# antrea-io/theia

Hardware: AMD Instinct MI355X
Metric: flow-records/sec (higher is better)
Workload: dtype u64 (aggregates) + f64 (detectors)

## Files before the change

### theia_amd/_capi.py

```python
import ctypes as C
import os

from . import build as _build

u64, i64, i32, u32, f64, f32 = C.c_uint64, C.c_int64, C.c_int32, C.c_uint32, C.c_double, C.c_float

TAD_ABI_VERSION = 13
TAD_KEY_SKIP = (1 << 64) - 1
TAD_OK = 0
TAD_ERR_INVALID_ARGUMENT, TAD_ERR_NO_DEVICE, TAD_ERR_OUT_OF_MEMORY, TAD_ERR_HIP = -1, -2, -3, -4
TAD_ERR_KEY_RANGE, TAD_ERR_GRID_TOO_LARGE, TAD_ERR_BUSY = -5, -6, -7
TAD_ALGO = {"EWMA": 0, "ARIMA": 1, "DBSCAN": 2, "DROP": 3}
TAD_AGG = {"": 0, None: 0, "None": 0, "pod": 1, "svc": 2, "external": 3}
TAD_OP = {"auto": 0, "max": 1, "sum": 2}
TAD_MEM_HOST, TAD_MEM_DEVICE = 0, 1
TAD_FLAG_EMIT_ALL_POINTS = 1
TAD_FLAG_KEY_U32, TAD_FLAG_TIME_U32 = 2, 4
TAD_KEY_SKIP32 = (1 << 32) - 1
TAD_FEATURE_NARROW_COLUMNS = 1
TAD_FEATURE_STREAM_DBSCAN = 2
TAD_STATE_HISTORY = 1
TAD_FEATURE_STREAM_ARIMA = 4
TAD_STATE_SERIES = 2
TAD_FEATURE_STREAM_TRIM = 8
TAD_STATE_TIMES = 8
TAD_FEATURE_STATE_RUN = 16
TAD_FEATURE_STATE_MERGE = 32
TAD_FEATURE_STATE_WINDOW = 64


class Plan(C.Structure):
    _fields_ = [("stage0", i32), ("partition_pass", i32), ("histogram", i32), ("sparse", i32), ("sparse_classes", i32),
                ("ewma_emit", i32), ("ewma_emit_rows", u32), ("reserved0", i32), ("tile_cells", i32), ("sparse_sort", i32), ("reserved1", i32)]


PLAN_VALUES = {
    "stage0": {"auto": 0, "v1": 1, "v2": 2}, "partition_pass": {"auto": 0, "sort": 1, "wc": 2, "wc_sectors": 3}, "histogram": {"auto": 0, "exact": 1, "sampled": 2},
    "sparse": {"auto": 0, "never": 1, "always": 2}, "sparse_classes": {"auto": 0, "always": 1}, "ewma_emit": {"auto": 0, "staged": 0, "lane": 1}, "tile_cells": {"auto": 0, "wide": 1},
    "sparse_sort": {"auto": 0, "lsd": 1, "partition": 2},
}


def make_plan(**kw):
    p = Plan()
    for name, v in kw.items():
        if name not in dict((f[0], 1) for f in Plan._fields_):
            raise ValueError("unknown tad_plan field %r" % name)
        if isinstance(v, str):
            v = PLAN_VALUES[name][v]
        setattr(p, name, int(v))
    return p


class KeyColumns(C.Structure):
    _fields_ = [("n_rows", u64), ("n_cols", i32), ("cols_a", C.POINTER(C.c_void_p)), ("keep_a", C.c_void_p),
                ("cols_b", C.POINTER(C.c_void_p)), ("keep_b", C.c_void_p), ("memory", C.c_int)]


class StringColumn(C.Structure):
    _fields_ = [("n_rows", u64), ("offsets", C.c_void_p), ("offset_bits", i32), ("data", C.c_void_p), ("data_bytes", u64),
                ("validity", C.c_void_p), ("validity_offset", u64), ("memory", C.c_int)]
# ... 136 lines not shown
```

### theia_amd/csrc/tad_capi.cpp

```cpp
#include "tad_engine.h"

using namespace tad;
using namespace tadh;

namespace tadh {

int ensure_rcp_table(JobCtx *e, uint64_t T) {
  const uint64_t want = T + 2;
  if (want <= e->rcp_n) return TAD_OK;
  uint64_t cap = want < 1024 ? 1024 : want + want / 4;
  int rc = ensure(e, e->rcp_table, cap * sizeof(double));
  if (rc != TAD_OK) return rc;
  std::vector<double> h(cap);
  h[0] = 0.0;
  for (uint64_t i = 1; i < cap; ++i) h[i] = 1.0 / (double)i;
  HIP_TRY(e, hipMemcpyAsync(e->rcp_table.p, h.data(), cap * sizeof(double), hipMemcpyHostToDevice, e->stream));
  HIP_TRY(e, hipStreamSynchronize(e->stream));
  e->rcp_n = cap;
  return TAD_OK;
}

int ensure_key_buffers(JobCtx *e, uint64_t K) {
  int rc;
  const uint64_t k = K ? K : 1;
// ... 24 lines not shown
    while (__atomic_load_n(&e->eng->pause_count, __ATOMIC_ACQUIRE) != 0 && std::chrono::steady_clock::now() - t0 < std::chrono::milliseconds(2))
      std::this_thread::sleep_for(std::chrono::microseconds(50));
    const uint32_t grace = __atomic_load_n(&e->eng->pause_count, __ATOMIC_ACQUIRE) != 0 ? 24u : 0u;
    if (relaunch(grace, &yielded_dev) != 0) return fail(e, TAD_ERR_HIP, "ARIMA launch failed");
    e->arima_relaunches++;
  }
  return TAD_OK;
}

int detect_and_count(JobCtx *e, Grid g, JobParams &jp, DevCounters *ctr, uint64_t *rows, bool stats_done = false) {
  hipStream_t s = e->stream;
  int rc;
  if ((rc = ensure_key_buffers(e, g.K)) != TAD_OK) return rc;
  if ((rc = ensure_rcp_table(e, g.T)) != TAD_OK) return rc;
  double *sigma = static_cast<double *>(e->sigma.p);
  uint32_t *n_pts = static_cast<uint32_t *>(e->n_pts.p);
  uint32_t *n_anom = static_cast<uint32_t *>(e->n_anom.p);
  unsigned long long *off = static_cast<unsigned long long *>(e->off.p);

  const bool ewma = jp.algo == TAD_ALGO_EWMA;
  const bool drop = jp.algo == TAD_ALGO_DROP;
  const bool db_fused = jp.algo == TAD_ALGO_DBSCAN && !jp.all_points && !stats_done && dbscan_uses_list(g);
  jp.lazy_sigma = db_fused;
  if (drop) {
    if ((rc = ensure(e, e->calc, (g.K * g.T ? g.K * g.T : 1) * sizeof(double))) != TAD_OK) return rc;
    launch_drop(s, g, jp.drop_nsigma, jp.drop_min_samples, static_cast<double *>(e->calc.p), sigma, n_pts,
                static_cast<double *>(e->key_mean.p), static_cast<double *>(e->key_m2.p), ctr);
  } else if (!stats_done && !db_fused)
    launch_key_sigma(s, g, jp.alpha, ewma && !jp.all_points, static_cast<const double *>(e->rcp_table.p), sigma, n_pts, n_anom, ctr, static_cast<double *>(e->key_mean.p),
                     static_cast<double *>(e->key_m2.p));
  if (jp.algo == TAD_ALGO_DBSCAN) {
    if ((rc = ensure(e, e->aux, dbscan_scratch_bytes(g))) != TAD_OK) return rc;
    if (dbscan_uses_list(g)) {
      DbscanStats dst{nullptr, nullptr, nullptr, nullptr};
      if (db_fused) dst = DbscanStats{n_pts, n_anom, static_cast<double *>(e->key_mean.p), static_cast<double *>(e->key_m2.p)};
      if (launch_dbscan(s, g, jp.eps, jp.min_samples, e->aux.p, dst, jp.settled && db_fused) != 0)
        return fail(e, TAD_ERR_HIP, "DBSCAN launch failed");
    } else {
      return fail(e, TAD_ERR_GRID_TOO_LARGE, "DBSCAN: series of %llu buckets are not supported", (unsigned long long)g.T);
    }
  } else if (jp.algo == TAD_ALGO_ARIMA) {
    if ((rc = ensure(e, e->calc, g.K * g.T * sizeof(double))) != TAD_OK) return rc;
    const size_t wsb = arima_workspace_bytes(g);
    if ((rc = ensure(e, e->aux, wsb)) != TAD_OK) return rc;
    const bool held = e->hold && e->hold->held;
    if (held) e->hold->release();
    const unsigned int *yielded_dev = nullptr;
    if (launch_arima(s, g, sigma, n_pts, jp.maxiter, static_cast<double *>(e->calc.p), ctr, e->aux.p, wsb, e->eng->pause_dev, &yielded_dev) != 0)
      return fail(e, TAD_ERR_HIP, "ARIMA launch failed");
    if ((rc = arima_yield_loop(e, yielded_dev, [&](uint32_t grace, const unsigned int **yd) {
           return launch_arima_fit(s, g, sigma, n_pts, jp.maxiter, static_cast<double *>(e->calc.p), ctr, e->aux.p, e->eng->pause_dev, yd, grace);
         })) != TAD_OK)
      return rc;
    if (held) e->hold->acquire();
  }
  const uint32_t *cnt = n_anom;
  if (jp.all_points && jp.algo != TAD_ALGO_ARIMA && !drop) cnt = n_pts;
  else if (db_fused) {}
  else if (!ewma || jp.all_points) launch_count_flags(s, g, jp.all_points, n_anom);
  launch_scan_moments(s, cnt, off, g.K, static_cast<unsigned long long *>(e->scan_scratch.p), dev_total(e), n_pts,
                      static_cast<const double *>(e->key_mean.p), static_cast<const double *>(e->key_m2.p), dev_moments(e), db_fused ? ctr : nullptr);
  HIP_TRY(e, hipMemcpyAsync(e->tail_host, e->counters.p, kTailBytes, hipMemcpyDeviceToHost, s));
  HIP_TRY(e, hipStreamSynchronize(s));
  HIP_TRY(e, hipGetLastError());
  *rows = *e->total_host;
  return TAD_OK;
}

}

namespace tadh {

void emit_rows(JobCtx *e, Grid g, Lattice L, const JobParams &jp, OutRows out, uint64_t rows) {
  const int kind = jp.algo == TAD_ALGO_EWMA ? 0 : (jp.algo == TAD_ALGO_ARIMA ? 1 : (jp.algo == TAD_ALGO_DROP ? 3 : (jp.lazy_sigma ? 4 : 2)));
  if (kind == 4 && !jp.all_points &&
      launch_emit_dbscan_list(e->stream, g, L, e->aux.p, static_cast<const uint32_t *>(e->n_anom.p), static_cast<const unsigned long long *>(e->off.p), out))
    return;
  launch_emit(e->stream, g, L, kind, jp.all_points, jp.alpha, static_cast<const double *>(e->sigma.p),
              static_cast<const uint32_t *>(e->n_pts.p), static_cast<const double *>(kind == 3 ? e->key_mean.p : e->calc.p),
              static_cast<const unsigned long long *>(e->off.p), out, rows, e->plan.ewma_emit, e->plan.ewma_emit_rows);
}

}

namespace {

int make_result(JobCtx *e, uint64_t rows, bool with_anomaly, tad_mem out_memory, ResultPriv **out, OutRows *dev_rows,
                ResultBlock *dev_block) {
  ResultPriv *rp = new (std::nothrow) ResultPriv();
  if (!rp) return fail(e, TAD_ERR_OUT_OF_MEMORY, "out of host memory");
  memset(rp, 0, sizeof *rp);
  const size_t bytes = result_bytes(rows, with_anomaly);
  int rc = alloc_device_block(e, bytes, dev_block);
  if (rc != TAD_OK) { delete rp; return rc; }
  carve(dev_block->base, rows, with_anomaly, dev_rows);
  rp->pub.n_rows = rows;
  rp->pub.memory = out_memory;
  *out = rp;
  return TAD_OK;
}
// ... 682 lines not shown
  HIP_TRY(e, hipEventRecord(e->ev[0], s));
  if (depth == 0) HIP_TRY(e, hipEventRecord(e->ev[6], s));
  int lat_mode = cols->n_buckets > 0 ? 0 : 1;
  Lattice L = make_lattice(cols->t0, lat_mode == 0 ? cols->step : 1, cols->n_buckets);
  bool empty = (n == 0 || K == 0);
  const tad_plan plan = e->plan;
  const bool force_v1 = plan.stage0 == 1;
  const bool force_v2 = plan.stage0 == 2;
  const bool has2 = cols->key_id2 != nullptr;
  bool force_v1_retry = false;
  bool force_wide_tiles = plan.tile_cells == 1;
  bool force_exact_hist = plan.histogram == 1;
  bool learnt_exact_hist = false, probing_sampled_hist = false;
  bool kh_rejected = false;
  bool sparse_lsd = plan.sparse_sort == 1;
  {
    const JobCtx::Learnt &lt = e->learnt;
    if (depth == 0 && lt.valid && lt.n == n && lt.K == K && lt.has2 == has2 && lt.algo == (int)job->algo && lt.op == (int)op_max) {
      if (lt.exact_hist) {
        if (lt.exact_uses >= lt.exact_backoff) probing_sampled_hist = true;
        else { force_exact_hist = true; learnt_exact_hist = true; }
      }
      if (lt.wide_tiles) force_wide_tiles = true;
    }
  }
  for (int attempt = 0; attempt < 11; ++attempt) {
    const bool hinted = lat_mode == 0;
    HIP_TRY(e, hipMemsetAsync(ctr, 0, kTailMoments, s));
    jp.settled = false;
    bool narrow_tiles = false;
    PartPlan pl{};
    bool v2 = !empty && !force_v1 && !force_v1_retry && (force_v2 || n >= (1ull << 22)) && part_plan_bins(n, K, has2, &pl);
    if (v2 && e->hold) e->hold->acquire();
    if ((rc = ensure(e, e->meta, sizeof(MetaPartial) * kMetaBlocks)) != TAD_OK) return rc;
    int meta_blocks = 0;
    bool hist_sampled = false;
    const tad_key_hist *kh = cols->key_hist;
    bool use_kh = v2 && depth == 0 && !kh_rejected && kh != nullptr && kh->bins != nullptr && lat_mode != 2 && kh->n_rows == n && kh->num_keys == K &&
                  kh->sides == (has2 ? 2u : 1u) && kh->workgroups == (uint32_t)pl.G && kh->nbins == pl.nbins && kh->shift == (uint32_t)pl.shift_bin &&
                  kh->chunk_rows == pl.chunk && rf.end_time == 0 && !(d_ts != nullptr && rf.start_time != 0);
    const uint32_t *binhist = nullptr;
    if (v2) {
      if ((rc = ensure(e, e->binhist, (size_t)pl.G * pl.nbins * 4)) != TAD_OK) return rc;
      hist_sampled = launch_meta_hist(s, (const uint64_t *)d_key, (const uint64_t *)d_key2, (const int64_t *)d_te, (const int64_t *)d_ts, n, K, rf,
                                      pl, static_cast<MetaPartial *>(e->meta.p), static_cast<uint32_t *>(e->binhist.p), ctr, cw,
                                      use_kh ||
// ... 495 lines not shown
        for (uint64_t i = 0; i < rows; ++i) st.n_anomalies += a[i];
      }
    }
    hipEventElapsedTime(&st.ms_meta, e->ev[0], e->ev[1]);
    hipEventElapsedTime(&st.ms_stage0, e->ev[1], e->ev[5]);
    hipEventElapsedTime(&st.ms_scatter, e->ev[2], e->ev[3]);
    hipEventElapsedTime(&st.ms_detect, e->ev[5], e->ev[4]);
    st.stage0_path = sparse ? (sp_part ? 8 : 4) : (v2 ? (pl.wc_cap ? 3 : 2) : 1);
    st.stage0_attempts = attempt + 1;
    st.hist_sampled = (v2 && hist_sampled) ? 1 : (use_kh ? 2 : 0);
    st.host_syncs = (hinted || empty) ? 2 : 3;
    st.job_context = e->index;
    st.arima_relaunches = e->arima_relaunches;
    hipEventElapsedTime(&st.ms_total, e->ev[0], e->ev[4]);
    if (depth == 0 && !points_mode && !stream) {
      JobCtx::Learnt &w = e->learnt;
      const bool exact_now = force_exact_hist && plan.histogram != 1;
      if (learnt_exact_hist) w.exact_uses++;
      else if (probing_sampled_hist) { w.exact_uses = 0; w.exact_backoff = exact_now ? (w.exact_backoff < 64 ? w.exact_backoff * 2 : 64) : 8; }
      else { w.exact_uses = 0; w.exact_backoff = 8; }
      w.valid = true; w.n = n; w.K = K; w.has2 = has2; w.algo = (int)job->algo; w.op = (int)op_max;
      w.exact_hist = exact_now;
      w.wide_tiles = force_wide_tiles && plan.tile_cells != 1;
    }
    strncpy(rp->pub.id, job->id, sizeof rp->pub.id - 1);
    if (stream && g.K) {
      unsigned long long added = 0;
      memcpy(&added, e->tail_host + kTailHistLen, 8);
      if (stream->history) stream->hist_len[stream->cur ^ 1] = stream->hist_len[stream->cur] + added;
      if (stream->series) stream->ser_len[stream->cur ^ 1] = stream->ser_len[stream->cur] + added;
      stream->cur ^= 1;
    }
    if (depth == 0) e->done.store(4);
    *out = &rp->pub;
    return TAD_OK;
  }
  return fail(e, TAD_ERR_HIP, "internal error: Stage 0 did not settle on a lattice / strategy after 6 attempts");
}

int sparse_points_direct(JobCtx *e, uint64_t n_rows_in, uint64_t rows_used, Lattice L, uint64_t P, DevCounters *ctr, tad_mem out_memory,
                         tad_points **points_out) {
  hipStream_t s = e->stream;
  int rc;
  if ((rc = ensure(e, e->counters, kTailBytes)) != TAD_OK) return rc;
  PointsPriv *pp = new (std::nothrow) PointsPriv();
  if (!pp) return fail(e, TAD_ERR_OUT_OF_MEMORY, "out of host memory");
// ... 828 lines not shown
```

### theia_amd/csrc/tad_engine.cpp

```cpp
#include "tad_engine.h"

using namespace tad;
using namespace tadh;

namespace tadh {

thread_local std::string g_static_err;

bool plan_ok(const tad_plan &p) {
  return p.stage0 >= 0 && p.stage0 <= 2 && p.partition_pass >= 0 && p.partition_pass <= 3 && p.histogram >= 0 && p.histogram <= 2 && p.sparse >= 0 &&
         p.sparse <= 2 && p.sparse_classes >= 0 && p.sparse_classes <= 1 && p.ewma_emit >= 0 && p.ewma_emit <= 1 && p.ewma_emit_rows <= 4096 && p.tile_cells >= 0 && p.tile_cells <= 1 && p.sparse_sort >= 0 && p.sparse_sort <= 2 && p.reserved0 == 0 && p.reserved1 == 0;
}

int vfail(tad_engine *e, int code, const char *fmt, va_list ap) {
  char buf[512];
  vsnprintf(buf, sizeof buf, fmt, ap);
  if (e) {
    std::lock_guard<std::mutex> lk(e->err_mu);
    e->err = buf;
  } else {
    g_static_err = buf;
  }
  return code;
}
int fail(tad_engine *e, int code, const char *fmt, ...) {
  va_list ap;
  va_start(ap, fmt);
  const int rc = vfail(e, code, fmt, ap);
  va_end(ap);
  return rc;
}
int fail(JobCtx *c, int code, const char *fmt, ...) {
  va_list ap;
  va_start(ap, fmt);
// ... 404 lines not shown
```

### theia_amd/csrc/tad_engine.h

```cpp
#ifndef THEIA_TAD_ENGINE_H
#define THEIA_TAD_ENGINE_H

#include <atomic>
#include <chrono>
#include <condition_variable>
#include <cstdarg>
#include <cstdio>
#include <cstdlib>
#include <cstring>
#include <mutex>
#include <new>
#include <string>
#include <thread>
#include <vector>

#include "tad_internal.h"

struct DevBuf {
  void *p = nullptr;
  size_t cap = 0;
};

struct FreeBlock {
  void *p;
// ... 21 lines not shown
  int *pause_dev = nullptr;
  hipStream_t signal_stream = nullptr;
  std::mutex pool_mu;
  std::vector<FreeBlock> free_blocks;
};

struct PauseHold;
struct JobCtx {
  tad_engine *eng = nullptr;
  PauseHold *hold = nullptr;
  int index = 0;
  bool busy = false;
  int device = 0;
  hipStream_t stream = nullptr;
  hipStream_t stream_normal = nullptr, stream_low = nullptr;
  bool own_streams = false;
  uint64_t ws_limit = 0;
  tad_plan plan{};
  std::atomic<int32_t> done{0}, total{0};
  char id[64] = {};
  DevBuf grid_val, grid_flag, sigma, n_pts, n_anom, off, scan_scratch, calc, counters, meta, aux, key_mean, key_m2;
  DevBuf in_key, in_key2, in_te, in_ts, in_val;
  DevBuf rcp_table;
  uint64_t rcp_n = 0;
  DevBuf binhist, part_total, part_start, part_offs32, recs, ovf, slices;
  DevBuf sp_comp_a, sp_comp_b, sp_val_a, sp_val_b, sp_temp, sp_first, sp_times;
  DevBuf sp_cls;
  DevBuf hs_key, hs_t, hs_val, hs_sorted, hs_noise, hs_cnt, hs_row, hs_koff, hs_kcnt;
  DevBuf wv_key, wv_pts;
  DevBuf mg_pts, mg_keys, mg_hist;
  struct MergeCall *merge = nullptr;
  DevBuf as_key, as_pt, as_ser, as_fit, as_pos, as_ws;
  int arima_relaunches = 0;
  bool sp_by_partition = false;
  DevBuf part_fin;
  DevBuf ovf_keys;
  hipEvent_t ev[8] = {};
  tad::MetaPartial *meta_host = nullptr;
  unsigned char *tail_host = nullptr;
  tad::DevCounters *ctr_host = nullptr;
  unsigned long long *total_host = nullptr;
  tad::Moments *moments_host = nullptr;
  struct Learnt {
    bool valid = false;
    uint64_t n = 0, K = 0;
    bool has2 = false;
    int algo = 0, op = 0;
    bool exact_hist = false;
    uint32_t exact_uses = 0, exact_backoff = 8;
    bool wide_tiles = false;
  } learnt;
};

struct MergeCall {
  int64_t keep_from = 0;
  tad_merge_stats stats{};
  bool changed = false;
  uint64_t added = 0;
};

struct tad_state {
  uint64_t K = 0;
  void *block[2] = {nullptr, nullptr};
  int cur = 0;
  bool history = false;
  unsigned long long *hist_off[2] = {nullptr, nullptr};
  unsigned long long *hist_val[2] = {nullptr, nullptr};
  uint64_t hist_cap[2] = {0, 0};
  uint64_t hist_len[2] = {0, 0};
  bool series = false;
  unsigned long long *ser_off[2] = {nullptr, nullptr};
  unsigned long long *ser_val[2] = {nullptr, nullptr};
  uint64_t ser_cap[2] = {0, 0};
// ... 38 lines not shown

constexpr int kMetaBlocks = 2048;
constexpr int kSampleBlockShift = 7;
constexpr int kDefaultJobsInFlight = 4;
constexpr int kMaxJobsInFlight = 16;
constexpr uint32_t kOverflowCap = 1u << 20;

bool plan_ok(const tad_plan &p);
int fail(tad_engine *e, int code, const char *fmt, ...);
int fail(JobCtx *c, int code, const char *fmt, ...);
int fail(std::nullptr_t, int code, const char *fmt, ...);

#define HIP_TRY(e, call)                                                                         \
  do {                                                                                           \
    hipError_t err__ = (call);                                                                   \
    if (err__ != hipSuccess)                                                                     \
      return fail((e), err__ == hipErrorOutOfMemory ? TAD_ERR_OUT_OF_MEMORY : TAD_ERR_HIP,       \
                  "%s failed: %s (%s:%d)", #call, hipGetErrorString(err__), __FILE__, __LINE__); \
  } while (0)


template <typename F> void for_each_buf(JobCtx *c, F f) {
  DevBuf *bufs[] = {&c->grid_val, &c->grid_flag, &c->sigma, &c->n_pts, &c->n_anom, &c->off, &c->scan_scratch, &c->calc, &c->counters, &c->meta, &c->aux,
                    &c->key_mean, &c->key_m2, &c->rcp_table, &c->binhist, &c->part_total, &c->part_start, &c->part_offs32, &c->recs, &c->ovf, &c->slices,
                    &c->sp_comp_a, &c->sp_comp_b, &c->sp_val_a, &c->sp_val_b, &c->sp_temp, &c->sp_first, &c->sp_times, &c->sp_cls, &c->part_fin, &c->ovf_keys,
                    &c->in_key, &c->in_key2, &c->in_te, &c->in_ts, &c->in_val,
                    &c->hs_key, &c->hs_t, &c->hs_val, &c->hs_sorted, &c->hs_noise, &c->hs_cnt, &c->hs_row, &c->hs_koff, &c->hs_kcnt,
                    &c->mg_pts, &c->mg_keys, &c->mg_hist,
                    &c->wv_key, &c->wv_pts,
                    &c->as_key, &c->as_pt, &c->as_ser, &c->as_fit, &c->as_pos, &c->as_ws};
  for (DevBuf *b : bufs) f(*b);
}

void drop_buffers(JobCtx *c);
void trim_idle(tad_engine *eng, JobCtx *self);
int ensure(JobCtx *e, DevBuf &b, size_t bytes);
void preload_code_objects();
JobCtx *ctx_create(tad_engine *eng, bool first);
void ctx_destroy(JobCtx *c);

struct Lease {
  tad_engine *eng;
  JobCtx *c = nullptr;
  Lease(tad_engine *eng_, const char *id = nullptr, bool low_priority = false) : eng(eng_) {
    std::unique_lock<std::mutex> lk(eng->mu);
    for (;;) {
      for (JobCtx *x : eng->ctxs)
// ... 51 lines not shown
void carve(void *base, uint64_t rows, bool with_anomaly, OutRows *o);
int alloc_device_block(JobCtx *e, size_t bytes, ResultBlock *rb);

struct ResultPriv {
  tad_result pub;
  void *block;
  size_t block_cap;
};

struct PointsPriv {
  tad_points pub;
  void *block;
  size_t block_cap;
};

struct JobParams {
  tad_algo algo;
  double alpha, eps;
  int min_samples, maxiter;
  double drop_nsigma;
  int drop_min_samples;
  bool all_points;
  bool lazy_sigma = false;
  bool settled = false;
};

int ensure_rcp_table(JobCtx *e, uint64_t T);
int ensure_key_buffers(JobCtx *e, uint64_t K);
void emit_rows(JobCtx *e, Grid g, Lattice L, const JobParams &jp, OutRows out, uint64_t rows = 0);

}

#endif
```

### theia_amd/csrc/tad_internal.h

```cpp
#pragma once
#include <hip/hip_runtime.h>
#include <stdint.h>
#include <type_traits>

#include "tad.h"

namespace tad {

struct Lattice {
  int64_t t0;
  int64_t step;
  uint64_t nb;
  uint64_t magic;
  int mode;
};

struct Grid {
  unsigned long long *val;
  uint8_t *flag;
  uint64_t K;
  uint64_t T;
  const long long *times;
};

// ... 172 lines not shown
  return r;
}

#endif

void launch_key_sigma(hipStream_t s, Grid g, double alpha, bool ewma_count, const double *rcp, double *sigma,
                      uint32_t *n_pts, uint32_t *n_anom, DevCounters *ctr, double *key_mean, double *key_m2);
static constexpr int kMomentBlocks = 128;
void launch_moments(hipStream_t s, uint64_t K, const uint32_t *n_pts, const double *key_mean,
                    const double *key_m2, Moments *partials, DevCounters *ctr = nullptr);
void launch_count_flags(hipStream_t s, Grid g, bool all_points, uint32_t *n_anom);
void launch_scan(hipStream_t s, const uint32_t *cnt, unsigned long long *off, uint64_t K,
                 unsigned long long *scratch, unsigned long long *total_copy = nullptr);
size_t scan_scratch_elems(uint64_t K);
void launch_scan_moments(hipStream_t s, const uint32_t *cnt, unsigned long long *off, uint64_t K, unsigned long long *scratch,
                         unsigned long long *total_copy, const uint32_t *n_pts, const double *key_mean, const double *key_m2, Moments *partials,
                         DevCounters *ctr);
void launch_emit(hipStream_t s, Grid g, Lattice lat, int kind, bool all_points, double alpha,
                 const double *sigma, const uint32_t *n_pts, const double *calc,
                 const unsigned long long *off, OutRows out, uint64_t rows_hint = 0,
                 int ewma_emit = 0, uint32_t ewma_emit_rows = 0);
void launch_emit_points(hipStream_t s, Grid g, Lattice lat, const unsigned long long *off, unsigned long long *out_key,
                        long long *out_t, unsigned long long *out_val);
struct StreamState {
  uint32_t *n;
  double *avg, *m2, *ewma;
  long long *last_t;
  unsigned char *seen;
};
struct StreamAcc {
  uint32_t n;
  double cnt, avg, m2, e;
  long long last_t;
  bool seen;
};

__device__ __forceinline__ StreamAcc stream_load(const StreamState &cur, uint64_t k) {
  const uint32_t n = cur.n[k];
  return StreamAcc{n, (double)n, cur.avg[k], cur.m2[k], cur.ewma[k], cur.last_t[k], cur.seen[k] != 0};
}

__device__ __forceinline__ void stream_store(const StreamState &next, uint64_t k, const StreamAcc &a) {
  next.n[k] = a.n; next.avg[k] = a.avg; next.m2[k] = a.m2; next.ewma[k] = a.e; next.last_t[k] = a.last_t; next.seen[k] = a.seen ? 1 : 0;
}

__device__ __forceinline__ bool stream_step(StreamAcc &a, double alpha, double one_minus, double x, long long ts, double *sg) {
// ... 290 lines not shown
```

### theia_amd/csrc/tad_kernels.hip

```cpp
#include <cstdlib>

#include "tad_internal.h"

namespace tad {

static constexpr int kBlock = 256;

__device__ __forceinline__ uint64_t gcd_u64(uint64_t a, uint64_t b) {
  if (a == 0) return b;
  if (b == 0) return a;
  if (((a | b) >> 32) == 0) {
    uint32_t x = (uint32_t)a, y = (uint32_t)b;
    while (y) { uint32_t r = x % y; x = y; y = r; }
    return x;
  }
  while (b) { uint64_t r = a % b; a = b; b = r; }
  return a;
}

__device__ __forceinline__ uint64_t absdiff_i64(int64_t a, int64_t b) {
  return a >= b ? (uint64_t)a - (uint64_t)b : (uint64_t)b - (uint64_t)a;
}

struct MetaAcc {
// ... 590 lines not shown
            reinterpret_cast<double2 *>(out.stddev + pos)[0] = ss;
            reinterpret_cast<double2 *>(out.stddev + pos)[1] = ss;
          }
          if (ALL) *reinterpret_cast<uint32_t *>(out.anomaly + pos) = (uint32_t)bv[0] | ((uint32_t)bv[1] << 8) | ((uint32_t)bv[2] << 16) | ((uint32_t)bv[3] << 24);
          pos += 4;
          nb = 0;
        }
      }
    }
  };
  if (COOP) walk_series_coop(g, k, [](uint64_t) {}, [&](uint64_t t, uint8_t fl, double x, int) { point(t, fl, x); });
  else walk_series(g, k, [&](uint64_t t, uint8_t fl, unsigned long long raw) { if (fl & FLAG_PRESENT) point(t, fl, (double)raw); });
#pragma unroll
  for (int i = 0; i < 3; ++i)
    if (i < nb) write_row(pos + i, bt[i], bx[i], ba[i], ALL && bv[i] != 0);
  if (LAZY) {
    sg = has_sigma ? sqrt(s_m2 / (s_cnt - 1.0)) : 0.0;
    if (COOP) { for (unsigned long long at = first + (threadIdx.x & 63); at < end; at += 64) out.stddev[at] = sg; }
    else { for (unsigned long long at = first; at < end; ++at) out.stddev[at] = sg; }
  }
}

static constexpr int kStageMarkTBits = 26;
__global__ __launch_bounds__(64) void k_emit_staged(Grid g, Lattice L, double alpha, const double *__restrict__ sigma,
                                                    const uint32_t *__restrict__ n_pts,
                                                    const unsigned long long *__restrict__ off, OutRows out, uint32_t cap) {
  extern __shared__ __attribute__((aligned(16))) unsigned char smem_stage[];
  double *s_e = reinterpret_cast<double *>(smem_stage);
  double *s_sg = s_e + cap;
  uint32_t *s_m = reinterpret_cast<uint32_t *>(s_sg + 64);
  const uint32_t lane = threadIdx.x;
  const uint64_t k0 = (uint64_t)blockIdx.x * 64;
  const uint64_t k = k0 + lane;
  const uint64_t kend = k0 + 64 < g.K ? k0 + 64 : g.K;
  const unsigned long long base = off[k0];
  const unsigned long long total = off[kend] - base;
  if (total == 0) return;
  const bool live = k < g.K;
  unsigned long long pos = live ? off[k] - base : 0;
  const unsigned long long end = live ? off[k + 1] - base : 0;
  const double sg = live ? sigma[k] : 0.0;
  s_sg[lane] = sg;
  if (pos != end) {
    const double one_minus = 1.0 - alpha;
    double e = 0.0;
    walk_series(g, k, [&](uint64_t t, uint8_t fl, unsigned long long raw) {
      if (!(fl & FLAG_PRESENT)) return;
      const double x = (double)raw;
      e = one_minus * e + alpha * x;
      if (fabs(x - e) > sg && pos < end) {
        if (pos < cap) {
          s_e[pos] = e;
          s_m[pos] = (lane << kStageMarkTBits) | (uint32_t)t;
        } else {
          const unsigned long long at = base + pos;
          out.key_id[at] = k;
          out.flow_end_s[at] = g.times != nullptr ? g.times[t * g.K + k] : (long long)(L.t0 + (int64_t)t * L.step);
          out.throughput[at] = x;
          out.algo_calc[at] = e;
          out.stddev[at] = sg;
        }
        pos++;
      }
    });
  }
  __syncthreads();
  const unsigned long long staged = total < cap ? total : cap;
  for (unsigned long long r = lane; r < staged; r += 64) {
    const uint32_t m = s_m[r];
    const uint32_t ln = m >> kStageMarkTBits;
    const uint64_t t = m & ((1u << kStageMarkTBits) - 1u);
    const uint64_t cell = t * g.K + (k0 + ln);
    const unsigned long long at = base + r;
    out.key_id[at] = k0 + ln;
    out.flow_end_s[at] = g.times != nullptr ? g.times[cell] : (long long)(L.t0 + (int64_t)t * L.step);
    out.throughput[at] = (double)g.val[cell];
    out.algo_calc[at] = s_e[r];
    out.stddev[at] = s_sg[ln];
  }
}

static uint32_t emit_stage_rows(uint64_t K, uint64_t rows_hint, int ewma_emit, uint32_t ewma_emit_rows) {
  if (ewma_emit == 1) return 0;
  uint64_t cap = 1536;
  if (rows_hint != 0) {
    const uint64_t mean = (rows_hint * 64 + K - 1) / K;
    cap = mean + mean / 8 + 128;
  }
  if (ewma_emit_rows != 0) cap = ewma_emit_rows;
  cap = (cap + 63) & ~63ull;
  if (cap < 64) cap = 64;
  if (cap > 4096) cap = 4096;
  return (uint32_t)cap;
}

void launch_emit(hipStream_t s, Grid g, Lattice lat, int kind, bool all_points, double alpha,
                 const double *sigma, const uint32_t *n_pts, const double *calc,
                 const unsigned long long *off, OutRows out, uint64_t rows_hint, int ewma_emit, uint32_t ewma_emit_rows) {
  if (g.K == 0) return;
  if (coop_shape(g)) {
    const int cblocks = (int)((g.K * 64 + kBlock - 1) / kBlock);
#define TAD_LAUNCH_EMIT_C(KIND, ALL) \
// ... 4 lines not shown
      if (kind == 0) TAD_LAUNCH_EMIT_C(0, false); else if (kind == 1) TAD_LAUNCH_EMIT_C(1, false); else if (kind == 3) TAD_LAUNCH_EMIT_C(3, false);
      else if (kind == 4) TAD_LAUNCH_EMIT_C(4, false); else TAD_LAUNCH_EMIT_C(2, false);
    }
#undef TAD_LAUNCH_EMIT_C
    return;
  }
  if (kind == 0 && !all_points && g.T < (1ull << kStageMarkTBits)) {
    if (const uint32_t cap = emit_stage_rows(g.K, rows_hint, ewma_emit, ewma_emit_rows)) {
      const unsigned blocks64 = (unsigned)((g.K + 63) / 64);
      hipLaunchKernelGGL(k_emit_staged, dim3(blocks64), dim3(64), (size_t)cap * 12 + 64 * 8, s, g, lat, alpha, sigma, n_pts, off, out, cap);
      return;
    }
  }
  const int blocks = (int)((g.K + kBlock - 1) / kBlock);
#define TAD_LAUNCH_EMIT(KIND, ALL) \
  hipLaunchKernelGGL((k_emit<KIND, ALL>), dim3(blocks), dim3(kBlock), 0, s, g, lat, alpha, sigma, n_pts, calc, off, out)
  if (all_points) {
    if (kind == 0) TAD_LAUNCH_EMIT(0, true); else if (kind == 1) TAD_LAUNCH_EMIT(1, true); else if (kind == 3) TAD_LAUNCH_EMIT(3, true); else TAD_LAUNCH_EMIT(2, true);
  } else {
    if (kind == 0) TAD_LAUNCH_EMIT(0, false); else if (kind == 1) TAD_LAUNCH_EMIT(1, false); else if (kind == 3) TAD_LAUNCH_EMIT(3, false);
    else if (kind == 4) TAD_LAUNCH_EMIT(4, false); else TAD_LAUNCH_EMIT(2, false);
  }
#undef TAD_LAUNCH_EMIT
}

__global__ __launch_bounds__(kBlock) void k_emit_points(Grid g, Lattice L, const unsigned long long *__restrict__ off,
                                                        unsigned long long *__restrict__ out_key, long long *__restrict__ out_t,
                                                        unsigned long long *__restrict__ out_val) {
  const uint64_t k = (uint64_t)blockIdx.x * kBlock + threadIdx.x;
  if (k >= g.K) return;
  unsigned long long pos = off[k];
  const unsigned long long end = off[k + 1];
  auto step = [&](uint64_t t, uint8_t fl, unsigned long long raw) {
    if ((fl & FLAG_PRESENT) && pos < end) {
      out_key[pos] = k;
      out_t[pos] = g.times != nullptr ? g.times[t * g.K + k] : (long long)(L.t0 + (int64_t)t * L.step);
      out_val[pos] = raw;
      pos++;
    }
  };
  uint64_t t = 0;
  for (; t + kUnroll <= g.T && pos < end; t += kUnroll) {
    uint8_t fl[kUnroll];
    unsigned long long v[kUnroll];
#pragma unroll
    for (int u = 0; u < kUnroll; ++u) { fl[u] = g.flag[(t + u) * g.K + k]; v[u] = g.val[(t + u) * g.K + k]; }
// ... 157 lines not shown
```

Measured before the change: 75.91 billion.

## Stage EWMA anomalies during counting and copy them at emit time

For EWMA without all-points output, a new count kernel computes per-key statistics, walks the EWMA once, and stages the anomalous rows (EWMA value plus a packed key/time mark) into a per-64-key global buffer. A block-level scan over the per-block row counts then replaces the per-key scan. The emit kernel rebuilds per-key offsets with a wave scan and reorders the staged rows through LDS instead of re-walking the series. It falls back to recomputing the rows when a block overflows the staging cap. This trades extra global staging memory and a more complex packed-mark path (13-bit anomaly index limits) for skipping a second series walk during emit.

Result: no change. 76.05 billion (median of 3 runs) (+0.2%).

```diff
diff --git a/theia_amd/_capi.py b/theia_amd/_capi.py
--- a/theia_amd/_capi.py
+++ b/theia_amd/_capi.py
@@ -36,7 +36,7 @@
 
 PLAN_VALUES = {
     "stage0": {"auto": 0, "v1": 1, "v2": 2}, "partition_pass": {"auto": 0, "sort": 1, "wc": 2, "wc_sectors": 3}, "histogram": {"auto": 0, "exact": 1, "sampled": 2},
-    "sparse": {"auto": 0, "never": 1, "always": 2}, "sparse_classes": {"auto": 0, "always": 1}, "ewma_emit": {"auto": 0, "staged": 0, "lane": 1}, "tile_cells": {"auto": 0, "wide": 1},
+    "sparse": {"auto": 0, "never": 1, "always": 2}, "sparse_classes": {"auto": 0, "always": 1}, "ewma_emit": {"auto": 0, "staged": 0, "lane": 1, "walk": 2}, "tile_cells": {"auto": 0, "wide": 1},
     "sparse_sort": {"auto": 0, "lsd": 1, "partition": 2},
 }
 
diff --git a/theia_amd/csrc/tad_capi.cpp b/theia_amd/csrc/tad_capi.cpp
--- a/theia_amd/csrc/tad_capi.cpp
+++ b/theia_amd/csrc/tad_capi.cpp
@@ -70,10 +70,20 @@
   const bool drop = jp.algo == TAD_ALGO_DROP;
   const bool db_fused = jp.algo == TAD_ALGO_DBSCAN && !jp.all_points && !stats_done && dbscan_uses_list(g);
   jp.lazy_sigma = db_fused;
+  jp.ewma_stage_cap = 0;
   if (drop) {
     if ((rc = ensure(e, e->calc, (g.K * g.T ? g.K * g.T : 1) * sizeof(double))) != TAD_OK) return rc;
     launch_drop(s, g, jp.drop_nsigma, jp.drop_min_samples, static_cast<double *>(e->calc.p), sigma, n_pts,
                 static_cast<double *>(e->key_mean.p), static_cast<double *>(e->key_m2.p), ctr);
+  } else if (!stats_done && ewma && !jp.all_points && e->plan.ewma_emit == 0 && ewma_stage_shape(g)) {
+    const uint32_t cap = ewma_stage_cap(g.K, g.T, jp.ewma_rows_hint, e->plan.ewma_emit_rows);
+    if ((rc = ensure(e, e->ewma_stage, ewma_stage_bytes(g.K, cap))) != TAD_OK) return rc;
+    const EwmaStage st = ewma_stage_view(e->ewma_stage.p, g.K, cap);
+    launch_ewma_count_stage(s, g, jp.alpha, static_cast<const double *>(e->rcp_table.p), sigma, n_pts, n_anom, ctr, static_cast<double *>(e->key_mean.p),
+                            static_cast<double *>(e->key_m2.p), st);
+    launch_scan_blocks_moments(s, st, off, g.K, dev_total(e), n_pts, static_cast<const double *>(e->key_mean.p), static_cast<const double *>(e->key_m2.p),
+                               dev_moments(e));
+    jp.ewma_stage_cap = cap;
   } else if (!stats_done && !db_fused)
     launch_key_sigma(s, g, jp.alpha, ewma && !jp.all_points, static_cast<const double *>(e->rcp_table.p), sigma, n_pts, n_anom, ctr, static_cast<double *>(e->key_mean.p),
                      static_cast<double *>(e->key_m2.p));
@@ -106,8 +116,9 @@
   if (jp.all_points && jp.algo != TAD_ALGO_ARIMA && !drop) cnt = n_pts;
   else if (db_fused) {}
   else if (!ewma || jp.all_points) launch_count_flags(s, g, jp.all_points, n_anom);
-  launch_scan_moments(s, cnt, off, g.K, static_cast<unsigned long long *>(e->scan_scratch.p), dev_total(e), n_pts,
-                      static_cast<const double *>(e->key_mean.p), static_cast<const double *>(e->key_m2.p), dev_moments(e), db_fused ? ctr : nullptr);
+  if (jp.ewma_stage_cap == 0)
+    launch_scan_moments(s, cnt, off, g.K, static_cast<unsigned long long *>(e->scan_scratch.p), dev_total(e), n_pts,
+                        static_cast<const double *>(e->key_mean.p), static_cast<const double *>(e->key_m2.p), dev_moments(e), db_fused ? ctr : nullptr);
   HIP_TRY(e, hipMemcpyAsync(e->tail_host, e->counters.p, kTailBytes, hipMemcpyDeviceToHost, s));
   HIP_TRY(e, hipStreamSynchronize(s));
   HIP_TRY(e, hipGetLastError());
@@ -124,6 +135,11 @@
   if (kind == 4 && !jp.all_points &&
       launch_emit_dbscan_list(e->stream, g, L, e->aux.p, static_cast<const uint32_t *>(e->n_anom.p), static_cast<const unsigned long long *>(e->off.p), out))
     return;
+  if (jp.ewma_stage_cap != 0) {
+    launch_emit_copy(e->stream, g, L, jp.alpha, static_cast<const double *>(e->sigma.p), static_cast<const uint32_t *>(e->n_anom.p),
+                     static_cast<unsigned long long *>(e->off.p), out, ewma_stage_view(e->ewma_stage.p, g.K, jp.ewma_stage_cap));
+    return;
+  }
   launch_emit(e->stream, g, L, kind, jp.all_points, jp.alpha, static_cast<const double *>(e->sigma.p),
               static_cast<const uint32_t *>(e->n_pts.p), static_cast<const double *>(kind == 3 ? e->key_mean.p : e->calc.p),
               static_cast<const unsigned long long *>(e->off.p), out, rows, e->plan.ewma_emit, e->plan.ewma_emit_rows);
@@ -852,6 +868,7 @@
         else { force_exact_hist = true; learnt_exact_hist = true; }
       }
       if (lt.wide_tiles) force_wide_tiles = true;
+      jp.ewma_rows_hint = lt.ewma_rows;
     }
   }
   for (int attempt = 0; attempt < 11; ++attempt) {
@@ -1393,6 +1410,7 @@
       w.valid = true; w.n = n; w.K = K; w.has2 = has2; w.algo = (int)job->algo; w.op = (int)op_max;
       w.exact_hist = exact_now;
       w.wide_tiles = force_wide_tiles && plan.tile_cells != 1;
+      w.ewma_rows = jp.algo == TAD_ALGO_EWMA && !jp.all_points ? rows : 0;
     }
     strncpy(rp->pub.id, job->id, sizeof rp->pub.id - 1);
     if (stream && g.K) {
diff --git a/theia_amd/csrc/tad_engine.cpp b/theia_amd/csrc/tad_engine.cpp
--- a/theia_amd/csrc/tad_engine.cpp
+++ b/theia_amd/csrc/tad_engine.cpp
@@ -9,7 +9,7 @@
 
 bool plan_ok(const tad_plan &p) {
   return p.stage0 >= 0 && p.stage0 <= 2 && p.partition_pass >= 0 && p.partition_pass <= 3 && p.histogram >= 0 && p.histogram <= 2 && p.sparse >= 0 &&
-         p.sparse <= 2 && p.sparse_classes >= 0 && p.sparse_classes <= 1 && p.ewma_emit >= 0 && p.ewma_emit <= 1 && p.ewma_emit_rows <= 4096 && p.tile_cells >= 0 && p.tile_cells <= 1 && p.sparse_sort >= 0 && p.sparse_sort <= 2 && p.reserved0 == 0 && p.reserved1 == 0;
+         p.sparse <= 2 && p.sparse_classes >= 0 && p.sparse_classes <= 1 && p.ewma_emit >= 0 && p.ewma_emit <= 2 && p.ewma_emit_rows <= 4096 && p.tile_cells >= 0 && p.tile_cells <= 1 && p.sparse_sort >= 0 && p.sparse_sort <= 2 && p.reserved0 == 0 && p.reserved1 == 0;
 }
 
 int vfail(tad_engine *e, int code, const char *fmt, va_list ap) {
diff --git a/theia_amd/csrc/tad_engine.h b/theia_amd/csrc/tad_engine.h
--- a/theia_amd/csrc/tad_engine.h
+++ b/theia_amd/csrc/tad_engine.h
@@ -67,6 +67,7 @@
   DevBuf grid_val, grid_flag, sigma, n_pts, n_anom, off, scan_scratch, calc, counters, meta, aux, key_mean, key_m2;
   DevBuf in_key, in_key2, in_te, in_ts, in_val;
   DevBuf rcp_table;
+  DevBuf ewma_stage;
   uint64_t rcp_n = 0;
   DevBuf binhist, part_total, part_start, part_offs32, recs, ovf, slices;
   DevBuf sp_comp_a, sp_comp_b, sp_val_a, sp_val_b, sp_temp, sp_first, sp_times;
@@ -94,6 +95,7 @@
     bool exact_hist = false;
     uint32_t exact_uses = 0, exact_backoff = 8;
     bool wide_tiles = false;
+    uint64_t ewma_rows = 0;
   } learnt;
 };
 
@@ -178,7 +180,7 @@
 
 template <typename F> void for_each_buf(JobCtx *c, F f) {
   DevBuf *bufs[] = {&c->grid_val, &c->grid_flag, &c->sigma, &c->n_pts, &c->n_anom, &c->off, &c->scan_scratch, &c->calc, &c->counters, &c->meta, &c->aux,
-                    &c->key_mean, &c->key_m2, &c->rcp_table, &c->binhist, &c->part_total, &c->part_start, &c->part_offs32, &c->recs, &c->ovf, &c->slices,
+                    &c->key_mean, &c->key_m2, &c->rcp_table, &c->ewma_stage, &c->binhist, &c->part_total, &c->part_start, &c->part_offs32, &c->recs, &c->ovf, &c->slices,
                     &c->sp_comp_a, &c->sp_comp_b, &c->sp_val_a, &c->sp_val_b, &c->sp_temp, &c->sp_first, &c->sp_times, &c->sp_cls, &c->part_fin, &c->ovf_keys,
                     &c->in_key, &c->in_key2, &c->in_te, &c->in_ts, &c->in_val,
                     &c->hs_key, &c->hs_t, &c->hs_val, &c->hs_sorted, &c->hs_noise, &c->hs_cnt, &c->hs_row, &c->hs_koff, &c->hs_kcnt,
@@ -276,6 +278,8 @@
   int drop_min_samples;
   bool all_points;
   bool lazy_sigma = false;
+  uint64_t ewma_rows_hint = 0;
+  uint32_t ewma_stage_cap = 0;
   bool settled = false;
 };
 
diff --git a/theia_amd/csrc/tad_internal.h b/theia_amd/csrc/tad_internal.h
--- a/theia_amd/csrc/tad_internal.h
+++ b/theia_amd/csrc/tad_internal.h
@@ -218,6 +218,23 @@
                  int ewma_emit = 0, uint32_t ewma_emit_rows = 0);
 void launch_emit_points(hipStream_t s, Grid g, Lattice lat, const unsigned long long *off, unsigned long long *out_key,
                         long long *out_t, unsigned long long *out_val);
+struct EwmaStage {
+  double *e;
+  unsigned long long *bbase;
+  uint32_t *m;
+  uint32_t *brows;
+  uint32_t cap;
+};
+bool ewma_stage_shape(const Grid &g);
+uint32_t ewma_stage_cap(uint64_t K, uint64_t T, uint64_t rows_hint, uint32_t ewma_emit_rows);
+size_t ewma_stage_bytes(uint64_t K, uint32_t cap);
+EwmaStage ewma_stage_view(void *ws, uint64_t K, uint32_t cap);
+void launch_ewma_count_stage(hipStream_t s, Grid g, double alpha, const double *rcp, double *sigma, uint32_t *n_pts, uint32_t *n_anom,
+                             DevCounters *ctr, double *key_mean, double *key_m2, EwmaStage st);
+void launch_scan_blocks_moments(hipStream_t s, EwmaStage st, unsigned long long *off, uint64_t K, unsigned long long *total_copy,
+                                const uint32_t *n_pts, const double *key_mean, const double *key_m2, Moments *partials);
+void launch_emit_copy(hipStream_t s, Grid g, Lattice lat, double alpha, const double *sigma, const uint32_t *n_anom, unsigned long long *off,
+                      OutRows out, EwmaStage st);
 struct StreamState {
   uint32_t *n;
   double *avg, *m2, *ewma;
diff --git a/theia_amd/csrc/tad_kernels.hip b/theia_amd/csrc/tad_kernels.hip
--- a/theia_amd/csrc/tad_kernels.hip
+++ b/theia_amd/csrc/tad_kernels.hip
@@ -636,25 +636,29 @@
 }
 
 static constexpr int kStageMarkTBits = 26;
-__global__ __launch_bounds__(64) void k_emit_staged(Grid g, Lattice L, double alpha, const double *__restrict__ sigma,
-                                                    const uint32_t *__restrict__ n_pts,
-                                                    const unsigned long long *__restrict__ off, OutRows out, uint32_t cap) {
-  extern __shared__ __attribute__((aligned(16))) unsigned char smem_stage[];
-  double *s_e = reinterpret_cast<double *>(smem_stage);
-  double *s_sg = s_e + cap;
-  uint32_t *s_m = reinterpret_cast<uint32_t *>(s_sg + 64);
+
+__device__ __forceinline__ void staged_rows_store(const Grid g, const Lattice L, OutRows out, unsigned long long base, uint64_t k0,
+                                                  unsigned long long staged, const double *s_e, const double *s_sg, const uint32_t *s_m) {
+  for (unsigned long long r = threadIdx.x; r < staged; r += 64) {
+    const uint32_t m = s_m[r];
+    const uint32_t ln = m >> kStageMarkTBits;
+    const uint64_t t = m & ((1u << kStageMarkTBits) - 1u);
+    const uint64_t cell = t * g.K + (k0 + ln);
+    const unsigned long long at = base + r;
+    out.key_id[at] = k0 + ln;
+    out.flow_end_s[at] = g.times != nullptr ? g.times[cell] : (long long)(L.t0 + (int64_t)t * L.step);
+    out.throughput[at] = (double)g.val[cell];
+    out.algo_calc[at] = s_e[r];
+    out.stddev[at] = s_sg[ln];
+  }
+}
+
+__device__ __forceinline__ void emit_staged_block(const Grid g, const Lattice L, double alpha, double sg, unsigned long long base,
+                                                  unsigned long long total, unsigned long long pos, unsigned long long end, OutRows out,
+                                                  uint32_t cap, double *s_e, const double *s_sg, uint32_t *s_m) {
   const uint32_t lane = threadIdx.x;
   const uint64_t k0 = (uint64_t)blockIdx.x * 64;
   const uint64_t k = k0 + lane;
-  const uint64_t kend = k0 + 64 < g.K ? k0 + 64 : g.K;
-  const unsigned long long base = off[k0];
-  const unsigned long long total = off[kend] - base;
-  if (total == 0) return;
-  const bool live = k < g.K;
-  unsigned long long pos = live ? off[k] - base : 0;
-  const unsigned long long end = live ? off[k + 1] - base : 0;
-  const double sg = live ? sigma[k] : 0.0;
-  s_sg[lane] = sg;
   if (pos != end) {
     const double one_minus = 1.0 - alpha;
     double e = 0.0;
@@ -679,19 +683,29 @@
     });
   }
   __syncthreads();
-  const unsigned long long staged = total < cap ? total : cap;
-  for (unsigned long long r = lane; r < staged; r += 64) {
-    const uint32_t m = s_m[r];
-    const uint32_t ln = m >> kStageMarkTBits;
-    const uint64_t t = m & ((1u << kStageMarkTBits) - 1u);
-    const uint64_t cell = t * g.K + (k0 + ln);
-    const unsigned long long at = base + r;
-    out.key_id[at] = k0 + ln;
-    out.flow_end_s[at] = g.times != nullptr ? g.times[cell] : (long long)(L.t0 + (int64_t)t * L.step);
-    out.throughput[at] = (double)g.val[cell];
-    out.algo_calc[at] = s_e[r];
-    out.stddev[at] = s_sg[ln];
-  }
+  staged_rows_store(g, L, out, base, k0, total < cap ? total : cap, s_e, s_sg, s_m);
+}
+
+__global__ __launch_bounds__(64) void k_emit_staged(Grid g, Lattice L, double alpha, const double *__restrict__ sigma,
+                                                    const uint32_t *__restrict__ n_pts,
+                                                    const unsigned long long *__restrict__ off, OutRows out, uint32_t cap) {
+  extern __shared__ __attribute__((aligned(16))) unsigned char smem_stage[];
+  double *s_e = reinterpret_cast<double *>(smem_stage);
+  double *s_sg = s_e + cap;
+  uint32_t *s_m = reinterpret_cast<uint32_t *>(s_sg + 64);
+  const uint32_t lane = threadIdx.x;
+  const uint64_t k0 = (uint64_t)blockIdx.x * 64;
+  const uint64_t k = k0 + lane;
+  const uint64_t kend = k0 + 64 < g.K ? k0 + 64 : g.K;
+  const unsigned long long base = off[k0];
+  const unsigned long long total = off[kend] - base;
+  if (total == 0) return;
+  const bool live = k < g.K;
+  const unsigned long long pos = live ? off[k] - base : 0;
+  const unsigned long long end = live ? off[k + 1] - base : 0;
+  const double sg = live ? sigma[k] : 0.0;
+  s_sg[lane] = sg;
+  emit_staged_block(g, L, alpha, sg, base, total, pos, end, out, cap, s_e, s_sg, s_m);
 }
 
 static uint32_t emit_stage_rows(uint64_t K, uint64_t rows_hint, int ewma_emit, uint32_t ewma_emit_rows) {
@@ -742,6 +756,207 @@
     else if (kind == 4) TAD_LAUNCH_EMIT(4, false); else TAD_LAUNCH_EMIT(2, false);
   }
 #undef TAD_LAUNCH_EMIT
+}
+
+static constexpr int kCountMarkBits = 13;
+
+bool ewma_stage_shape(const Grid &g) { return g.K != 0 && !coop_shape(g) && (g.T + 1) * 8 <= 32768; }
+
+uint32_t ewma_stage_cap(uint64_t K, uint64_t T, uint64_t rows_hint, uint32_t ewma_emit_rows) {
+  uint64_t cap = emit_stage_rows(K, rows_hint, 0, ewma_emit_rows);
+  const uint64_t lds_max = ((65536 - (T + 1) * 8) / 12) & ~63ull, grid_max = (48 * T) & ~63ull;
+  if (cap > lds_max) cap = lds_max;
+  if (cap > grid_max) cap = grid_max;
+  return (uint32_t)(cap < 64 ? 64 : cap);
+}
+
+size_t ewma_stage_bytes(uint64_t K, uint32_t cap) {
+  const uint64_t nb = (K + 63) / 64;
+  return (size_t)(nb * cap * 12 + (nb + 1) * 8 + nb * 4);
+}
+
+EwmaStage ewma_stage_view(void *ws, uint64_t K, uint32_t cap) {
+  const uint64_t nb = (K + 63) / 64;
+  EwmaStage st;
+  st.e = static_cast<double *>(ws);
+  st.bbase = reinterpret_cast<unsigned long long *>(st.e + nb * cap);
+  st.m = reinterpret_cast<uint32_t *>(st.bbase + nb + 1);
+  st.brows = st.m + nb * cap;
+  st.cap = cap;
+  return st;
+}
+
+__global__ __launch_bounds__(64) void k_ewma_count_stage(Grid g, double alpha, const double *__restrict__ rcp_g, double *__restrict__ sigma,
+                                                         uint32_t *__restrict__ n_pts, uint32_t *__restrict__ n_anom, DevCounters *ctr,
+                                                         double *__restrict__ key_mean, double *__restrict__ key_m2, EwmaStage st) {
+  extern __shared__ __attribute__((aligned(16))) unsigned char smem_count[];
+  const uint32_t cap = st.cap;
+  double *s_e = reinterpret_cast<double *>(smem_count);
+  double *rcp = s_e + cap;
+  uint32_t *s_m = reinterpret_cast<uint32_t *>(rcp + g.T + 1);
+  const uint32_t lane = threadIdx.x;
+  const uint64_t k0 = (uint64_t)blockIdx.x * 64;
+  const bool live = k0 + lane < g.K;
+  const uint64_t k = live ? k0 + lane : g.K - 1;
+  for (uint64_t i = lane; i <= g.T; i += 64) rcp[i] = rcp_g[i];
+  __syncthreads();
+  double cnt = 0.0, avg = 0.0, m2 = 0.0;
+  uint32_t n = 0;
+  walk_series(g, k, [&](uint64_t, uint8_t fl, unsigned long long raw) {
+    if (fl & FLAG_PRESENT) {
+      const double x = (double)raw;
+      cnt = cnt + 1.0;
+      n++;
+      const double d = x - avg;
+      const double dn = div_by_count(d, cnt, rcp[n]);
+      avg = avg + dn;
+      m2 = m2 + d * (d - dn);
+    }
+  });
+  const bool has_sigma = n >= 2;
+  const double sg = has_sigma ? sqrt(m2 / (cnt - 1.0)) : 0.0;
+  const bool judged = live && has_sigma;
+  const double one_minus = 1.0 - alpha;
+  double e = 0.0;
+  uint32_t a = 0, cursor = 0;
+  walk_series(g, k, [&](uint64_t t, uint8_t fl, unsigned long long raw) {
+    const bool present = (fl & FLAG_PRESENT) != 0;
+    const double x = (double)raw;
+    const double en = one_minus * e + alpha * x;
+    e = present ? en : e;
+    const bool anom = judged && present && fabs(x - e) > sg;
+    const unsigned long long hits = __ballot(anom);
+    if (anom) {
+      const uint32_t at = cursor + __builtin_amdgcn_mbcnt_hi((uint32_t)(hits >> 32), __builtin_amdgcn_mbcnt_lo((uint32_t)hits, 0u));
+      if (at < cap) {
+        s_e[at] = e;
+        s_m[at] = (lane << kStageMarkTBits) | (a << kCountMarkBits) | (uint32_t)t;
+      }
+      a++;
+    }
+    cursor += (uint32_t)__popcll(hits);
+  });
+  unsigned long long my_pts = 0;
+  unsigned my_key = 0;
+  if (live) {
+    sigma[k] = sg;
+    n_pts[k] = n;
+    if (key_mean != nullptr) { key_mean[k] = avg; key_m2[k] = m2; }
+    n_anom[k] = a;
+    my_pts = n;
+    my_key = n > 0;
+  }
+  if (lane == 0) st.brows[blockIdx.x] = cursor;
+  __syncthreads();
+  if (cursor <= cap) {
+    const uint64_t slot = (uint64_t)blockIdx.x * cap;
+    for (uint32_t r = lane; r < cursor; r += 64) {
+      st.e[slot + r] = s_e[r];
+      st.m[slot + r] = s_m[r];
+    }
+  }
+  for (int d = 32; d >= 1; d >>= 1) {
+    my_pts += __shfl_down(my_pts, d);
+    my_key += __shfl_down(my_key, d);
+  }
+  if (lane == 0 && my_key) {
+    atomicAdd(&ctr->n_points, my_pts);
+    atomicAdd(&ctr->n_keys, (unsigned long long)my_key);
+  }
+}
+
+void launch_ewma_count_stage(hipStream_t s, Grid g, double alpha, const double *rcp, double *sigma, uint32_t *n_pts, uint32_t *n_anom,
+                             DevCounters *ctr, double *key_mean, double *key_m2, EwmaStage st) {
+  const unsigned blocks64 = (unsigned)((g.K + 63) / 64);
+  hipLaunchKernelGGL(k_ewma_count_stage, dim3(blocks64), dim3(64), (size_t)st.cap * 12 + (size_t)(g.T + 1) * 8, s, g, alpha, rcp, sigma, n_pts, n_anom,
+                     ctr, key_mean, key_m2, st);
+}
+
+__global__ __launch_bounds__(kBlock) void k_scan_blocks(const uint32_t *__restrict__ brows, uint32_t nb, unsigned long long *__restrict__ bbase,
+                                                        unsigned long long *total_out, unsigned long long *total_copy, MomentsArgs M) {
+  if (blockIdx.x != 0) {
+    moments_block(blockIdx.x - 1, M.K, M.n_pts, M.key_mean, M.key_m2, M.partials, M.ctr);
+    return;
+  }
+  unsigned long long carry = 0;
+  for (uint64_t tile = 0; tile < nb; tile += kScanTile) {
+    const uint64_t i0 = tile + (uint64_t)threadIdx.x * kScanItems;
+    uint32_t c[kScanItems];
+    unsigned long long sum = 0;
+    for (int j = 0; j < kScanItems; ++j) {
+      c[j] = i0 + j < nb ? brows[i0 + j] : 0u;
+      sum += c[j];
+    }
+    unsigned long long tot;
+    unsigned long long ex = block_exclusive_scan(sum, &tot) + carry;
+    for (int j = 0; j < kScanItems; ++j) {
+      if (i0 + j < nb) bbase[i0 + j] = ex;
+      ex += c[j];
+    }
+    carry += tot;
+  }
+  if (threadIdx.x == 0) {
+    bbase[nb] = carry;
+    *total_out = carry;
+    if (total_copy != nullptr) *total_copy = carry;
+  }
+}
+
+void launch_scan_blocks_moments(hipStream_t s, EwmaStage st, unsigned long long *off, uint64_t K, unsigned long long *total_copy,
+                                const uint32_t *n_pts, const double *key_mean, const double *key_m2, Moments *partials) {
+  const MomentsArgs M{K, n_pts, key_mean, key_m2, partials, nullptr};
+  hipLaunchKernelGGL(k_scan_blocks, dim3(1 + kMomentBlocks), dim3(kBlock), 0, s, st.brows, (uint32_t)((K + 63) / 64), st.bbase, off + K, total_copy, M);
+}
+
+__global__ __launch_bounds__(64) void k_emit_copy(Grid g, Lattice L, double alpha, const double *__restrict__ sigma,
+                                                  const uint32_t *__restrict__ n_anom, unsigned long long *__restrict__ off, OutRows out,
+                                                  EwmaStage st) {
+  extern __shared__ __attribute__((aligned(16))) unsigned char smem_copy[];
+  const uint32_t cap = st.cap;
+  double *s_e = reinterpret_cast<double *>(smem_copy);
+  double *s_sg = s_e + cap;
+  uint32_t *s_m = reinterpret_cast<uint32_t *>(s_sg + 64);
+  uint32_t *s_off = s_m + cap;
+  const uint32_t lane = threadIdx.x;
+  const uint64_t k0 = (uint64_t)blockIdx.x * 64;
+  const uint64_t k = k0 + lane;
+  const bool live = k < g.K;
+  const unsigned long long base = st.bbase[blockIdx.x];
+  const unsigned long long total = st.bbase[blockIdx.x + 1] - base;
+  const uint32_t a = live ? n_anom[k] : 0u;
+  uint32_t incl = a;
+  for (int d = 1; d < 64; d <<= 1) {
+    const uint32_t y = __shfl_up(incl, d);
+    if (lane >= (uint32_t)d) incl += y;
+  }
+  const uint32_t pos = incl - a;
+  if (live) off[k] = base + pos;
+  if (total == 0) return;
+  const double sg = live ? sigma[k] : 0.0;
+  s_sg[lane] = sg;
+  if (total > cap) {
+    emit_staged_block(g, L, alpha, sg, base, total, pos, (unsigned long long)pos + a, out, cap, s_e, s_sg, s_m);
+    return;
+  }
+  s_off[lane] = pos;
+  __syncthreads();
+  const uint64_t slot = (uint64_t)blockIdx.x * cap;
+  constexpr uint32_t low = (1u << kCountMarkBits) - 1u;
+  for (uint32_t r = lane; r < (uint32_t)total; r += 64) {
+    const uint32_t m = st.m[slot + r];
+    const uint32_t ln = m >> kStageMarkTBits;
+    const uint32_t at = s_off[ln] + ((m >> kCountMarkBits) & low);
+    s_e[at] = st.e[slot + r];
+    s_m[at] = (ln << kStageMarkTBits) | (m & low);
+  }
+  __syncthreads();
+  staged_rows_store(g, L, out, base, k0, total, s_e, s_sg, s_m);
+}
+
+void launch_emit_copy(hipStream_t s, Grid g, Lattice lat, double alpha, const double *sigma, const uint32_t *n_anom, unsigned long long *off,
+                      OutRows out, EwmaStage st) {
+  const unsigned blocks64 = (unsigned)((g.K + 63) / 64);
+  hipLaunchKernelGGL(k_emit_copy, dim3(blocks64), dim3(64), (size_t)st.cap * 12 + 64 * 8 + 64 * 4, s, g, lat, alpha, sigma, n_anom, off, out, st);
 }
 
 __global__ __launch_bounds__(kBlock) void k_emit_points(Grid g, Lattice L, const unsigned long long *__restrict__ off,
```
